# kssteven418/Q-ASR

Measured on AMD Instinct MI355X. Metric: RTFx (audio-sec/wall-sec) QuartzNet15x5 int8 bs32, higher is better.
Workload: dtype int8 (s8 x s8 -> i32 on MFMA; float64 fixed-point requant)

## Files before the change

profiles/phase_stamps.py:

```python
#!/usr/bin/env python3
import argparse
import ctypes as C
import json
import os
import sys

ROOT = os.path.dirname(os.path.dirname(os.path.abspath(__file__)))
sys.path.insert(0, os.path.join(ROOT, 'q-asr_amd'))
sys.path.insert(0, ROOT)
import numpy as np
import torch

ap = argparse.ArgumentParser()
ap.add_argument('--tile', type=int, default=32, choices=[32, 64, 128])
ap.add_argument('--gen', type=int, default=2)
ap.add_argument('--batch', type=int, default=32)
args = ap.parse_args()
from qasr import engine, pack, synth, topology

d = np.load(os.path.join(ROOT, 'tests/golden/net_quartznet_w8a8.npz'))
meta = json.loads(str(d['meta']))
cfg = topology.quartznet15x5()
sd = synth.make_state_dict(cfg, meta['seed'])
blob, pm = pack.pack_model(cfg, sd, d['act_min'], d['act_max'], 8, 8)
e = engine.Engine(blob, 0, tile=args.tile, sep_gen=getattr(args, "gen", 2))
B, T = args.batch, 512
x = torch.from_numpy(synth.make_features(B, 64, T, 1)).cuda()
lens = torch.full((B,), 500)
for _ in range(3):
    e.forward(x, lens)
torch.cuda.synchronize()
lib = engine.load_library()
buf = torch.zeros(32, dtype=torch.int64, device='cuda')
lib.qasr_debug_prof(C.c_void_p(buf.data_ptr()))
labels = e.op_labels()
seen = {}
for oi, lab in enumerate(labels):
    if lab.startswith('k_sep'):
        seen[lab] = oi
for lab, oi in seen.items():
    for _ in range(3):
        e.run_op(oi)
    torch.cuda.synchronize()
    st = buf.cpu().numpy()
    n = int(st[31])
    deltas = [int(st[i + 1] - st[i]) for i in range(n - 1)]
    print(f'{lab:34s} op {oi:3d} stamps {n:2d} total {int(st[n - 1] - st[0]):6d}  deltas {deltas}')
lib.qasr_debug_prof(C.c_void_p(0))
e.close()
```

q-asr_amd/csrc/qasr_sep2_impl.h:

```cpp
#pragma once
#include <algorithm>
#include <cstdio>
#include <cstdlib>
#include <type_traits>

#include "qasr_device.h"

namespace qasr {

typedef int v2i __attribute__((ext_vector_type(2)));
typedef unsigned char __attribute__((address_space(3))) lds_u8;
typedef unsigned __attribute__((address_space(3))) lds_u32;
typedef v2i __attribute__((address_space(3))) lds_v2i;
typedef v4i __attribute__((address_space(3))) lds_v4i;

#define SEP2_NT 512
#ifndef SEP2_WPE
#define SEP2_WPE 2
#endif
#define SEP2_CH 128

template <int K, int TT>
struct Sep2Geo {
  static constexpr int PAD = K / 2;
  static constexpr int HALO = (PAD + 15) / 16 * 16;
  static constexpr int D = HALO - PAD;
  static constexpr int NU = TT / 16;
  static constexpr int S = 4 * NU;
  static constexpr int MS = -(D & 3);
  static constexpr int NS = (K + 3 - MS + 3) / 4;
  static constexpr int A0 = D + MS;
  static constexpr int RG = S < 16 ? S : 16;
  static constexpr int OFF = (A0 & (RG - 1)) / 4;
  static constexpr int NE = OFF + NU + NS - 1;
  static constexpr int NRD = (4 * NE + RG - 1) / RG;
  static constexpr int WLEN = TT + 2 * HALO;
#ifndef SEP2_CF128
#define SEP2_CF128 1
#endif
  static constexpr int WP = (TT > 64 && !SEP2_CF128) ? WLEN : ((WLEN + 4 * S - 1) / (4 * S) | 1) * (4 * S);
  static constexpr int NPG = WLEN / 16;
  static constexpr int NPT = (16 * NPG + 63) / 64;
  static constexpr int KP4 = (K + 3) / 4;
  static constexpr int KS = 4 * KP4 + 32;
  static constexpr int TAPB = 16 * KS;
  static constexpr int NTT = (KS + 63) / 64;
  static constexpr int WREG = 16 * WP + TAPB + 64;
  static_assert(3 * S + (A0 & ~(RG - 1)) + NRD * RG <= WLEN && WLEN <= WP, "lane stream leaves the window row");
  static_assert(8 + MS - 3 >= 0 && 8 + MS + 4 * (NS + 1) <= KS, "tap stream leaves the tap row");
  static_assert(WREG % 16 == 0, "wave regions are not 16-byte granular");
};

__device__ __forceinline__ int rq_clamp(int z, double M, int lo, int hi) { return med3i(rq_rint(z, M), lo, hi); }
__device__ __forceinline__ unsigned pack4b(int a, int b, int c, int d) {
  const unsigned lo = __builtin_amdgcn_perm((unsigned)b, (unsigned)a, 0x0c0c0400u);
  const unsigned hi = __builtin_amdgcn_perm((unsigned)d, (unsigned)c, 0x04000c0cu);
  return lo | hi;
}

__device__ __forceinline__ int sep2_a_lane_off(int lane) {
  return (16 * (lane >> 5) + ((lane & 15) >> 1)) * 32 + 16 * ((lane >> 4) & 1) + 8 * (lane & 1);
}
__device__ __forceinline__ v4i sep2_a_frag(const lds_u8* img_lane, int ks) {
  const v2i lo = __builtin_amdgcn_ds_read_tr8_b64_v2i32((lds_v2i*)(img_lane + ks * 1024));
  const v2i hi = __builtin_amdgcn_ds_read_tr8_b64_v2i32((lds_v2i*)(img_lane + ks * 1024 + 256));
  return (v4i){lo[0], lo[1], hi[0], hi[1]};
}
__device__ __forceinline__ void sep2_load_wg(v4i* wb, const v4i* __restrict__ wp) {
#pragma unroll
  for (int i = 0; i < 4; ++i) wb[i] = wp[64 * i];
}
template <int MT, int N, int N0>
__device__ __forceinline__ void sep2_gemm(v16i (&acc)[MT], v4i (&wf)[16], const lds_u8* img_lane, int mt_stride,
                                          const v4i* __restrict__ r0, const v4i* __restrict__ r1) {
  constexpr int AB = MT > 2 ? 1 : 2;
  constexpr int NQ = 4 * N / AB;
  v4i a[2][MT][AB];
#pragma unroll
  for (int mt = 0; mt < MT; ++mt)
#pragma unroll
    for (int i = 0; i < AB; ++i) a[0][mt][i] = sep2_a_frag(img_lane + mt * mt_stride, i);
#pragma unroll
  for (int q = 0; q < NQ; ++q) {
    if (q + 1 < NQ) {
#pragma unroll
      for (int mt = 0; mt < MT; ++mt)
#pragma unroll
        for (int i = 0; i < AB; ++i) a[(q + 1) & 1][mt][i] = sep2_a_frag(img_lane + mt * mt_stride, AB * (q + 1) + i);
    }
#pragma unroll
    for (int i = 0; i < AB; ++i)
#pragma unroll
      for (int mt = 0; mt < MT; ++mt)
        acc[mt] = __builtin_amdgcn_mfma_i32_32x32x32_i8(a[q & 1][mt][i], wf[AB * q + i], acc[mt], 0, 0, 0);
    if ((AB * (q + 1)) % 4 == 0) {
      const int g = (AB * (q + 1)) / 4 - 1;
      if (g < N0) {
        if (r0) sep2_load_wg(&wf[4 * g], r0 + 256 * g);
      } else {
        if (r1) sep2_load_wg(&wf[4 * g], r1 + 256 * g);
      }
    }
  }
}

template <int D, int NE, int RG>
__device__ __forceinline__ void sep2_rd_stream(unsigned* xs, const lds_u8* wr) {
  if constexpr (D < NE) {
    constexpr int n = (RG == 16 && D % 4 == 0 && NE - D >= 4) ? 4 : (D % 2 == 0 && NE - D >= 2) ? 2 : 1;
    if constexpr (n == 4) {
      const v4i v = *(const lds_v4i*)(wr + 4 * D);
      xs[D] = v[0]; xs[D + 1] = v[1]; xs[D + 2] = v[2]; xs[D + 3] = v[3];
    } else if constexpr (n == 2) {
      const v2i v = *(const lds_v2i*)(wr + 4 * D);
      xs[D] = v[0]; xs[D + 1] = v[1];
    } else {
      xs[D] = *(const lds_u32*)(wr + 4 * D);
    }
    sep2_rd_stream<D + n, NE, RG>(xs, wr);
  }
}

__device__ __forceinline__ v4i sep2_mask16(v4i pk, int n) {
#pragma unroll
  for (int i = 0; i < 4; ++i) {
    const int m = min(max(n - 4 * i, 0), 4);
    pk[i] &= m >= 4 ? -1 : (int)((1u << (8 * m)) - 1u);
  }
  return pk;
}
template <int MT>
__device__ __forceinline__ bool sep2_any_wide(const v16i (&a)[MT]) {
  int mx = a[0][0], mn = a[0][0];
#pragma unroll
  for (int mt = 0; mt < MT; ++mt)
#pragma unroll
    for (int r = 0; r < 16; r += 2) {
      mx = max(max(mx, a[mt][r]), a[mt][r + 1]);
      mn = min(min(mn, a[mt][r]), a[mt][r + 1]);
    }
  return __any(mx >= (1 << 21) || mn < -(1 << 21));
}

template <int I, int N, class F>
__device__ __forceinline__ void sep2_for(F&& f) {
  if constexpr (I < N) {
    f(std::integral_constant<int, I>{});
    sep2_for<I + 1, N>(f);
  }
}
template <int MT, int N, int N0, int AB, class CB>
__device__ __forceinline__ void sep2_gemm_cb(v16i* __restrict__ acc, v4i (&wf)[16], const lds_u8* img_lane, int mt_stride,
                                             const v4i* __restrict__ r0, const v4i* __restrict__ r1, CB&& cb) {
  constexpr int NQ = 4 * N / AB;
  v4i a[2][MT][AB];
#pragma unroll
  for (int mt = 0; mt < MT; ++mt)
#pragma unroll
    for (int i = 0; i < AB; ++i) a[0][mt][i] = sep2_a_frag(img_lane + mt * mt_stride, i);
  sep2_for<0, NQ>([&](auto qc) {
    constexpr int q = decltype(qc)::value;
    if constexpr (q + 1 < NQ) {
#pragma unroll
      for (int mt = 0; mt < MT; ++mt)
#pragma unroll
        for (int i = 0; i < AB; ++i) a[(q + 1) & 1][mt][i] = sep2_a_frag(img_lane + mt * mt_stride, AB * (q + 1) + i);
    }
    sep2_for<0, AB * MT>([&](auto sc) {
      constexpr int sl = decltype(sc)::value, i = sl / MT, mt = sl % MT;
      acc[mt] = __builtin_amdgcn_mfma_i32_32x32x32_i8(a[q & 1][mt][i], wf[AB * q + i], acc[mt], 0, 0, 0);
      __builtin_amdgcn_sched_barrier(0);
      cb(std::integral_constant<int, q * AB * MT + sl>{});
      __builtin_amdgcn_sched_barrier(0);
    });
    if constexpr ((AB * (q + 1)) % 4 == 0) {
      constexpr int g = (AB * (q + 1)) / 4 - 1;
      if constexpr (g < N0) {
        if (r0) sep2_load_wg(&wf[4 * g], r0 + 256 * g);
      } else {
        if (r1) sep2_load_wg(&wf[4 * g], r1 + 256 * g);
      }
    }
    __builtin_amdgcn_sched_barrier(0);
  });
}

template <int MT, int J0, int NJ, class CB>
__device__ __forceinline__ void sep2_gemm_ks(v16i* __restrict__ acc, v4i (&wf)[16], const lds_u8* img_lane, int mt_stride, CB&& cb) {
  v4i a[2][MT];
#pragma unroll
  for (int mt = 0; mt < MT; ++mt) a[0][mt] = sep2_a_frag(img_lane + mt * mt_stride, J0);
  sep2_for<0, NJ>([&](auto qc) {
    constexpr int q = decltype(qc)::value;
    if constexpr (q + 1 < NJ) {
#pragma unroll
      for (int mt = 0; mt < MT; ++mt) a[(q + 1) & 1][mt] = sep2_a_frag(img_lane + mt * mt_stride, J0 + q + 1);
    }
    sep2_for<0, MT>([&](auto mc) {
      constexpr int mt = decltype(mc)::value;
      acc[mt] = __builtin_amdgcn_mfma_i32_32x32x32_i8(a[q & 1][mt], wf[J0 + q], acc[mt], 0, 0, 0);
      __builtin_amdgcn_sched_barrier(0);
      cb(std::integral_constant<int, q * MT + mt>{});
      __builtin_amdgcn_sched_barrier(0);
    });
    __builtin_amdgcn_sched_barrier(0);
  });
}

#define SEP2_PAIR_HALF 32768
#define SEP2_PAIR_SPIN 400000
typedef unsigned v4u __attribute__((ext_vector_type(4)));
typedef v4u __attribute__((address_space(3))) lds_v4u;
typedef unsigned __attribute__((address_space(1))) glb_u32;
__device__ __forceinline__ void sep2_pair_signal(unsigned* flag, int tid) {
  asm volatile("s_waitcnt vmcnt(0)" ::: "memory");
  __syncthreads();
  if (tid == 0) (void)__hip_atomic_fetch_add((glb_u32*)flag, 1u, __ATOMIC_RELAXED, __HIP_MEMORY_SCOPE_AGENT);
}
__device__ __forceinline__ void sep2_pair_wait(unsigned* flag, unsigned* tmo, int wave, int lane) {
  if (wave == 0) {
    const unsigned long long t_end = __builtin_amdgcn_s_memrealtime() + SEP2_PAIR_SPIN;
    while (__hip_atomic_load((glb_u32*)flag, __ATOMIC_RELAXED, __HIP_MEMORY_SCOPE_AGENT) == 0u) {
      __builtin_amdgcn_s_sleep(2);
      if (__builtin_amdgcn_s_memrealtime() > t_end) {
        if (lane == 0) (void)__hip_atomic_fetch_add((glb_u32*)tmo, 1u, __ATOMIC_RELAXED, __HIP_MEMORY_SCOPE_AGENT);
        break;
      }
    }
  }
  __builtin_amdgcn_fence(__ATOMIC_ACQUIRE, "wavefront");
  __syncthreads();
}

struct Sep2PassP {
  int bias, pbias;
  double Mo[QASR_MAX_OUTS];
  double Mm, Mp;
  float sbm, sbp;
};

template <int K, int NG, int NGP, int NP, bool DBG, int TT, int DIL = 1, bool SKIP = false, bool PAIR = false>
__device__ __forceinline__ void sep2_body(const SepP& p, const int b, const int t0, const bool stamp_wg, const int wg_id,
                                          const int hm = 0, const int pair_id = 0) {
  using G = Sep2Geo<K, TT / DIL>;
  constexpr bool RES = NGP > 0;
  static_assert(!PAIR || (K > 0 && NG == 4 && NGP == 0 && NP == 2 && !DBG && TT == 128 && DIL == 1 && !SKIP),
                "paired form: the plain 512 -> 512 layers at 128 frames");
  constexpr int NPL = PAIR ? 1 : NP;
  const int cbase = PAIR ? 256 * hm : 0;
  static_assert(DIL == 1 || (DIL == 2 && !RES && TT >= 64), "dilation 2: plain layers, 64- / 128-frame tiles");
  constexpr int MT = TT / 32;
  constexpr int NU = G::NU, S = G::S, NS = G::NS;
  constexpr int CIN_PAD = 128 * NG, PCIN_PAD = 128 * NGP;
  constexpr int RCH = 16 / DIL, GCH = SEP2_CH / DIL;
  constexpr int NCHUNK = PAIR ? 2 : (CIN_PAD + GCH - 1) / GCH;
  constexpr int NPGR = DIL == 1 ? G::NPG : (TT + 2 * DIL * G::HALO) / 16;
  constexpr int NPT = (RCH * NPGR + 63) / 64, NTG = RCH * G::KS / 16, NTT = (NTG + 63) / 64;
  static_assert(DIL == 1 || (8 * NPGR == G::WLEN && (RCH * G::KS) % 16 == 0), "dilation 2: window / tap granules");
  extern __shared__ __attribute__((aligned(16))) unsigned char smem[];
  const EpiP& e = p.e;
  int tid_ = threadIdx.x;
  asm volatile("" : "+v"(tid_));
  const int tid = tid_, lane = tid & 63, h = lane >> 5;
  const int wave = __builtin_amdgcn_readfirstlane(tid >> 6);
  lds_u8* const Xd = (lds_u8*)smem;
  lds_u8* const Un = Xd + TT * CIN_PAD;
  lds_u8* const Wsw = Un + wave * G::WREG;
  lds_u8* const Tlw = Wsw + 16 * G::WP;

  const unsigned flags = e.flags;
  const int eT = e.T, eTp = e.Tp, ecout = e.cout, n_outs = e.n_outs;
  const int len_b = e.lens[b];
  const int lim = (flags & QASR_F_MASK_OUT) ? min(len_b, eT) : eT;
  const int dlim = min(len_b, eT);
  const bool f_relu = flags & QASR_F_RELU;
  const bool f_exact = flags & QASR_F_EXACT_Z;
  int dw_lo = p.dw_lo, dw_hi = p.dw_hi;
  asm volatile("" : "+v"(dw_lo), "+v"(dw_hi));
  const bool stamp = p.prof && (p.prof_mode & 255) == 0 && stamp_wg && tid == 0;
  const bool tline = p.prof && (p.prof_mode & 255) == 1 && tid == 0;
  const int tune = p.prof_mode >> 8;
  long long tl_start = 0, tl_clk = 0;
  if (tline) {
    tl_start = (long long)__builtin_amdgcn_s_memrealtime();
    tl_clk = (long long)__builtin_amdgcn_s_memtime();
  }
  int nst = 0;
#define STAMP2() do { if (stamp && nst < 31) p.prof[nst++] = (long long)__builtin_amdgcn_s_memtime(); } while (0)
  STAMP2();

  const unsigned flip = p.x_unsigned ? 0x80808080u : 0u;
  constexpr int NRT = RES ? (TT * PCIN_PAD / 16) / SEP2_NT : 0;
  v4i pc[NPT], pt[NTT], rr[NRT > 0 ? NRT : 1], wf[16];
  const int co_l = 32 * wave + (lane & 31);
  const v4i* const w0 = w_frag(p.w, CIN_PAD, cbase + co_l, 0);
  const v4i* const w0a = PAIR ? w0 + 64 * 8 * hm : w0;
  const v4i* const w0b = PAIR ? w0 + 64 * 8 * (1 - hm) - 64 * 8 : w0;
  int woff[NPT], toff[NTT];
  unsigned wkeep[NPT];
  lds_u8* wlds[NPT];
#pragma unroll
  for (int i = 0; i < NPT; ++i) {
    const int pi = lane + 64 * i;
    const int row = pi / NPGR, col = pi - row * NPGR;
    const int t = t0 - DIL * G::HALO + 16 * col;
    woff[i] = min(row, RCH - 1) * eTp + min(max(t, 0), eTp - 16);
    wkeep[i] = (t >= 0 && t < eTp) ? 0xffffffffu : 0u;
    wlds[i] = DIL == 1 ? Wsw + min(row, 15) * G::WP + 16 * col : Wsw + 2 * min(row, RCH - 1) * G::WP + 8 * col;
    asm volatile("" : "+v"(wkeep[i]));
  }
#pragma unroll
  for (int i = 0; i < NTT; ++i) toff[i] = 16 * min(lane + 64 * i, NTG - 1);
  auto ld_grp = [&](int g) {
    const int cw = cbase + GCH * g + RCH * wave;
    const int8_t* const xg = p.x + ((size_t)b * CIN_PAD + cw) * eTp;
    const unsigned char* const tg = (const unsigned char*)p.wdw2 + (size_t)cw * G::KS;
#pragma unroll
    for (int i = 0; i < NPT; ++i) pc[i] = *(const v4i*)(xg + woff[i]);
#pragma unroll
    for (int i = 0; i < NTT; ++i) pt[i] = *(const v4i*)(tg + toff[i]);
  };
  auto ld_res = [&](int i) {
    if constexpr (RES) {
      const int gi = tid + SEP2_NT * i;
      const int c = gi / (TT / 16), q = gi - c * (TT / 16);
      rr[i] = *(const v4i*)(p.panes[0].x + ((size_t)b * PCIN_PAD + c) * eTp + t0 + 16 * q);
    }
  };
  constexpr int SLC = NCHUNK >= 4 ? 3 : PAIR ? 2 : 1;
  auto pf = [&](auto chc, int lo, int hi) {
    constexpr int CH = decltype(chc)::value;
    constexpr int n_res = CH + 1 == NCHUNK ? NRT : 0;
    constexpr int s0 = CH < SLC ? 4 * NG * CH / SLC : 0, n_slab = CH < SLC ? 4 * NG * (CH + 1) / SLC - s0 : 0;
#pragma unroll
    for (int i = lo; i < hi; ++i) {
      if (i < n_res) ld_res(i);
      else if (i < n_res + n_slab) wf[s0 + i - n_res] = (s0 + i - n_res < 8 ? w0a : w0b)[64 * (s0 + i - n_res)];
    }
  };
  auto commit = [&]() {
#pragma unroll
    for (int i = 0; i < NPT; ++i) {
      if (64 * i + 63 < RCH * NPGR || lane + 64 * i < RCH * NPGR) {
        v4i v = pc[i];
        v[0] = (v[0] & wkeep[i]) ^ flip; v[1] = (v[1] & wkeep[i]) ^ flip; v[2] = (v[2] & wkeep[i]) ^ flip; v[3] = (v[3] & wkeep[i]) ^ flip;
        if constexpr (DIL == 1) {
          *(lds_v4i*)wlds[i] = v;
        } else {
          const v2i ev = {(int)__builtin_amdgcn_perm((unsigned)v[1], (unsigned)v[0], 0x06040200u),
                          (int)__builtin_amdgcn_perm((unsigned)v[3], (unsigned)v[2], 0x06040200u)};
          const v2i od = {(int)__builtin_amdgcn_perm((unsigned)v[1], (unsigned)v[0], 0x07050301u),
                          (int)__builtin_amdgcn_perm((unsigned)v[3], (unsigned)v[2], 0x07050301u)};
          *(lds_v2i*)wlds[i] = ev;
          *(lds_v2i*)(wlds[i] + G::WP) = od;
        }
      }
    }
#pragma unroll
    for (int i = 0; i < NTT; ++i) {
      const int gi = lane + 64 * i;
      if (64 * i + 63 < NTG || gi < NTG) *(lds_v4i*)(Tlw + 16 * gi) = pt[i];
    }
  };
  constexpr int NXT = K == 0 ? (TT * CIN_PAD / 16) / SEP2_NT : 1;
  v4i xg[NXT];
  if constexpr (K == 0) {
#pragma unroll
    for (int i = 0; i < NXT; ++i) {
      const int gi = tid + SEP2_NT * i;
      const int c = gi / (TT / 16), q = gi - c * (TT / 16);
      xg[i] = *(const v4i*)(p.x + ((size_t)b * CIN_PAD + c) * eTp + t0 + 16 * q);
    }
#pragma unroll
    for (int j = 0; j < 4 * NG; ++j) wf[j] = w0[64 * j];
  } else {
    ld_grp(0);
  }
  STAMP2();

  const int cb = lane >> 2, jl = lane & 3;
  int dbias[NCHUNK];
  double dM[NCHUNK];
  if constexpr (K > 0) {
#pragma unroll
    for (int gi = 0; gi < NCHUNK; ++gi) {
      const int c = cbase + GCH * gi + RCH * wave + cb / DIL;
      dbias[gi] = p.bias_dw[c];
      dM[gi] = p.m_dw[c];
    }
  }
  Sep2PassP pps[NPL];
  auto load_pps = [&]() {
#pragma unroll
  for (int ps = 0; ps < NPL; ++ps) {
    const int cor = cbase + 256 * ps + co_l;
    Sep2PassP& q = pps[ps];
    q.bias = p.bias[cor];
    if constexpr (RES) {
      q.pbias = p.panes[0].bias[cor];
      q.Mm = e.m_main[cor];
      q.Mp = p.panes[0].m[cor];
      q.sbp = f_exact ? p.panes[0].sb[cor] : 1.0f;
    } else {
#pragma unroll
      for (int j = 0; j < QASR_MAX_OUTS; ++j) q.Mo[j] = j < n_outs ? e.outs[j].mtab[cor] : 0.0;
    }
    q.sbm = f_exact ? e.sb[cor] : 1.0f;
  }
  };
  if constexpr (K == 0) load_pps();

  if constexpr (SKIP && !DBG) {
    asm volatile("" ::: "memory");
    if ((flags & QASR_F_MASK_OUT) && t0 >= lim && !p.prof) {
      store_masked_tile<SEP2_NT>(e, b, t0, TT, 0, ecout, tid);
      return;
    }
  }
  const bool full_in = t0 + TT <= dlim;
  constexpr int e0base = 8 + G::MS;
  const int e0 = e0base - jl, tq = e0 >> 2, tsh = e0 & 3;
  unsigned fmask[NU];
  {
    const int dl = dlim - t0 - S * jl;
#pragma unroll
    for (int u = 0; u < NU; ++u) {
      const int n = min(max(dl - 4 * u, 0), 4);
      fmask[u] = n >= 4 ? 0xffffffffu : ((1u << (8 * n)) - 1u);
    }
  }
  struct DwIn {
    unsigned raw[NS + 1];
    unsigned xs[G::NRD * (G::RG / 4)];
  };
  const lds_u32* tr_lane = (const lds_u32*)(Tlw + (cb / DIL) * G::KS + 4 * tq);
  const lds_u8* wr_lane = Wsw + cb * G::WP + S * jl + (G::A0 & ~(G::RG - 1));
  asm volatile("" : "+v"(tr_lane), "+v"(wr_lane));
  auto dw_read = [&](DwIn& in) {
    const lds_u32* tr = tr_lane;
#pragma unroll
    for (int i = 0; i <= NS; ++i) in.raw[i] = tr[i];
    const lds_u8* wr = wr_lane;
    sep2_rd_stream<G::OFF, G::NE, G::RG>(in.xs, wr);
  };
  auto dw_mfma = [&](const DwIn& in, v4i (&acc)[NU], int bias, auto&& pf3) {
    unsigned tw[NS];
#pragma unroll
    for (int st = 0; st < NS; ++st) tw[st] = __builtin_amdgcn_alignbyte(in.raw[st + 1], in.raw[st], tsh);
#pragma unroll
    for (int u = 0; u < NU; ++u) acc[u] = (v4i){bias, bias, bias, bias};
    pf3(0);
#pragma unroll
    for (int st = 0; st < NS; ++st) {
      if (st == NS / 2) pf3(1);
#pragma unroll
      for (int u = 0; u < NU; ++u)
        acc[u] = __builtin_amdgcn_mfma_i32_4x4x4i8((int)tw[st], (int)in.xs[G::OFF + u + st], acc[u], 0, 0, 0);
    }
    pf3(2);
  };
  auto dw_out = [&](v4i (&acc)[NU], int c0, double Mg) {
    if constexpr (DIL == 2) {
      const int c = c0 + RCH * wave + (cb >> 1), par = cb & 1;
#pragma unroll
      for (int u = 0; u < NU; ++u)
#pragma unroll
        for (int v = 0; v < 4; ++v) {
          const int f = 2 * (S * jl + 4 * u + v) + par;
          if (DBG && p.dw_acc_dbg && t0 + f < eT) p.dw_acc_dbg[((size_t)b * CIN_PAD + c) * eTp + t0 + f] = acc[u][v];
          *(lds_u8*)(Xd + (f >> 5) * (CIN_PAD * 32) + c * 32 + (f & 31)) = (unsigned char)rq_clamp(acc[u][v], Mg, dw_lo, dw_hi);
        }
      return;
    }
    const int c = c0 + 16 * wave + cb;
    if (DBG && p.dw_acc_dbg) {
#pragma unroll
      for (int u = 0; u < NU; ++u)
#pragma unroll
        for (int v = 0; v < 4; ++v) {
          const int f = S * jl + 4 * u + v;
          if (t0 + f < eT) p.dw_acc_dbg[((size_t)b * CIN_PAD + c) * eTp + t0 + f] = acc[u][v];
        }
    }
#pragma unroll
    for (int u = 0; u < NU; ++u) {
      const int f = S * jl + 4 * u;
      const unsigned w = pack4b(rq_clamp(acc[u][0], Mg, dw_lo, dw_hi), rq_clamp(acc[u][1], Mg, dw_lo, dw_hi),
                                rq_clamp(acc[u][2], Mg, dw_lo, dw_hi), rq_clamp(acc[u][3], Mg, dw_lo, dw_hi));
      *(lds_u32*)(Xd + (f >> 5) * (CIN_PAD * 32) + c * 32 + (f & 31)) = w & fmask[u];
    }
  };

  auto dw_mfma_ilv = [&](const DwIn& in, v4i (&acc)[NU], int bias, auto&& pf3, v4i (&prev)[NU], int cprev, double Mprev) {
    constexpr int NOPS = 17 * NU, OPM = (NOPS + NS * NU - 1) / (NS * NU);
    const int c = cprev + 16 * wave + cb;
#pragma unroll
    for (int u = 0; u < NU; ++u) acc[u] = (v4i){bias, bias, bias, bias};
    unsigned tws[2] = {__builtin_amdgcn_alignbyte(in.raw[1], in.raw[0], tsh), 0u}, P1 = 0, P2 = 0;
    double dreg = 0.0;
    int q[4] = {0, 0, 0, 0};
    __builtin_amdgcn_sched_barrier(0);
    sep2_for<0, NS * NU>([&](auto ic) {
      constexpr int i = decltype(ic)::value, st = i / NU, u = i % NU;
      if constexpr (u == 0) {
        if constexpr (st == 0) pf3(0);
        if constexpr (st == NS / 2) pf3(1);
      }
      if constexpr (u == NU / 2 && st + 1 < NS) tws[(st + 1) & 1] = __builtin_amdgcn_alignbyte(in.raw[st + 2], in.raw[st + 1], tsh);
      acc[u] = __builtin_amdgcn_mfma_i32_4x4x4i8((int)tws[st & 1], (int)in.xs[G::OFF + u + st], acc[u], 0, 0, 0);
      sep2_for<OPM * i, OPM * (i + 1)>([&](auto jc) {
      constexpr int j = decltype(jc)::value;
      if constexpr (j < NOPS) {
        constexpr int dw = j / 17, r = j % 17;
        if constexpr (r < 12) {
          constexpr int val = r / 3, ph = r % 3;
          if constexpr (ph == 0) dreg = (double)prev[dw][val];
          if constexpr (ph == 1) dreg = __builtin_fma(dreg, Mprev, MAGIC_RNE);
          if constexpr (ph == 2) q[val] = med3i(__double2loint(dreg), dw_lo, dw_hi);
        } else if constexpr (r == 12) {
          P1 = __builtin_amdgcn_perm((unsigned)q[1], (unsigned)q[0], 0x0c0c0400u);
        } else if constexpr (r == 13) {
          P2 = __builtin_amdgcn_perm((unsigned)q[3], (unsigned)q[2], 0x04000c0cu);
        } else if constexpr (r == 14) {
          P1 |= P2;
        } else if constexpr (r == 15) {
          P1 &= fmask[dw];
        } else {
          constexpr int f0 = 4 * dw;
          const int f = S * jl + f0;
          *(lds_u32*)(Xd + (f >> 5) * (CIN_PAD * 32) + c * 32 + (f & 31)) = P1;
        }
      }
      });
      __builtin_amdgcn_sched_barrier(0);
    });
    pf3(2);
  };

  DwIn in;
  auto stage = [&](auto chc) {
    constexpr int CH = decltype(chc)::value;
    commit();
    if constexpr (CH + 1 < NCHUNK) ld_grp(CH + 1);
    __builtin_amdgcn_fence(__ATOMIC_RELEASE, "wavefront");
    __builtin_amdgcn_wave_barrier();
    __builtin_amdgcn_fence(__ATOMIC_ACQUIRE, "wavefront");
    dw_read(in);
    __builtin_amdgcn_sched_barrier(0);
  };
#ifndef SEP2_ILV
#define SEP2_ILV 1
#endif
#ifndef SEP2_TAIL1
#define SEP2_TAIL1 0
#endif
  constexpr bool ILV = SEP2_ILV && (!RES || TT <= 64) && DIL == 1;
  v4i accs[ILV ? 2 : 1][NU];
  auto chunk = [&](auto chc) {
    constexpr int CH = decltype(chc)::value;
    constexpr int c0 = GCH * CH;
    constexpr int NPF = (CH + 1 == NCHUNK ? NRT : 0) + (CH < SLC ? 4 * NG * (CH + 1) / SLC - 4 * NG * CH / SLC : 0);
    constexpr int Q = (NPF + 2) / 3;
    if constexpr (ILV) {
      if constexpr (CH == 0) dw_mfma(in, accs[0], dbias[0], [&](int k) { pf(chc, Q * k, Q * (k + 1)); });
      else {
        if (DBG && p.dw_acc_dbg) {
          dw_out(accs[(CH - 1) & 1], c0 - GCH, dM[CH - 1]);
          dw_mfma(in, accs[CH & 1], dbias[CH], [&](int k) { pf(chc, Q * k, Q * (k + 1)); });
        } else {
          dw_mfma_ilv(in, accs[CH & 1], dbias[CH], [&](int k) { pf(chc, Q * k, Q * (k + 1)); }, accs[(CH - 1) & 1],
                      c0 - GCH, dM[CH - 1]);
        }
      }
      __builtin_amdgcn_sched_barrier(0);
      STAMP2();
      if constexpr (CH + 1 < NCHUNK) stage(std::integral_constant<int, CH + 1>{});
      else dw_out(accs[CH & 1], c0, dM[CH]);
      STAMP2();
    } else {
      dw_mfma(in, accs[0], dbias[CH], [&](int k) { pf(chc, Q * k, Q * (k + 1)); });
      STAMP2();
      if constexpr (CH + 1 < NCHUNK) stage(std::integral_constant<int, CH + 1>{});
      dw_out(accs[0], c0, dM[CH]);
      __builtin_amdgcn_sched_barrier(0);
      STAMP2();
    }
  };
  if constexpr (K > 0) {
    if (stamp) {
      asm volatile("s_waitcnt vmcnt(0)" ::: "memory");
      STAMP2();
    }
    if (tune & 1) {
      if (wave < 4) __builtin_amdgcn_s_setprio(3);
    }
    stage(std::integral_constant<int, 0>{});
    load_pps();
    if (tune & 2) {
      if (wave >= 4)
        for (int i = 0; i < ((tune >> 4) & 127); ++i) __builtin_amdgcn_s_sleep(1);
    }
    STAMP2();
    sep2_for<0, NCHUNK>([&](auto chc) { chunk(chc); });
  } else {
    static_assert(K > 0 || !RES, "the bare 1x1 form has no residual variant");
    const unsigned xflip = p.pw_unsigned ? 0x80808080u : 0u;
#pragma unroll
    for (int i = 0; i < NXT; ++i) {
      const int gi = tid + SEP2_NT * i;
      const int c = gi / (TT / 16), q = gi - c * (TT / 16);
      v4i v = xg[i];
      v[0] ^= xflip; v[1] ^= xflip; v[2] ^= xflip; v[3] ^= xflip;
      *(lds_v4i*)(Xd + (q >> 1) * (CIN_PAD * 32) + c * 32 + 16 * (q & 1)) = v;
    }
  }
  static_assert(NCHUNK <= 4 * DIL, "more than 512 input channels");
  if ((tune & 5) == 1) __builtin_amdgcn_s_setprio(0);
  __syncthreads();
  if constexpr (PAIR) {
    const auto rs = __builtin_amdgcn_make_buffer_rsrc(p.pair_x + ((size_t)pair_id * 2 + hm) * SEP2_PAIR_HALF, 0, SEP2_PAIR_HALF, 0x00020000);
#pragma unroll
    for (int i = 0; i < MT; ++i) {
      const v4u v = *(const lds_v4u*)(Xd + i * (CIN_PAD * 32) + tid * 16);
      __builtin_amdgcn_raw_buffer_store_b128(v, rs, i * (SEP2_PAIR_HALF / MT) + tid * 16, 0, 16);
    }
  }
  if constexpr (DIL == 2) {
    if (t0 + TT > dlim) {
      for (int r = tid; r < MT * CIN_PAD; r += SEP2_NT) {
        const int mt = r / CIN_PAD, n = dlim - t0 - 32 * mt;
        if (n < 32) {
          lds_v4i* row = (lds_v4i*)(Xd + (size_t)r * 32);
          row[0] = sep2_mask16(row[0], n);
          row[1] = sep2_mask16(row[1], n - 16);
        }
      }
      __syncthreads();
    }
  }
  if constexpr (RES) {
    const unsigned rflip = p.panes[0].x_unsigned ? 0x80808080u : 0u;
#pragma unroll
    for (int i = 0; i < NRT; ++i) {
      const int gi = tid + SEP2_NT * i;
      const int c = gi / (TT / 16), q = gi - c * (TT / 16);
      v4i v = rr[i];
      v[0] ^= rflip; v[1] ^= rflip; v[2] ^= rflip; v[3] ^= rflip;
      *(lds_v4i*)(Un + (q >> 1) * (PCIN_PAD * 32) + c * 32 + 16 * (q & 1)) = v;
    }
    __syncthreads();
  }
  STAMP2();
  const lds_u8* const xd_lane = Xd + sep2_a_lane_off(lane);
  const lds_u8* const xr_lane = Un + sep2_a_lane_off(lane);
  int32_t* const pdbg = RES ? p.panes[0].acc_dbg : nullptr;
  const int qlo = f_relu ? max(e.qlo, 0) : e.qlo, qhi = e.qhi;
  constexpr bool PIPED = !RES && (NP * (MT >= 2 ? 2 : 1) > 1);
  static_assert(!PAIR || PIPED, "paired form: the pipelined epilogue");
  if constexpr (PIPED) {
    {
      constexpr int MH = MT >= 2 ? MT / 2 : 1, NH = MT / MH;
      constexpr bool SPLIT = SEP2_TAIL1 && MH == 2;
      constexpr int NUN0 = NP * NH, NUN = NUN0 + (SPLIT ? 1 : 0);
      const OutP& o0 = e.outs[0];
      const int olo = o0.lo, ohi = o0.hi;
      int8_t* const optr = (int8_t*)o0.ptr;
      v16i accs[2][MH];
      int q4[4];
      unsigned P[4];
      auto unit_finish = [&](v16i* a, int ps, int mt0, auto mhc) __attribute__((always_inline)) {
        constexpr int mh = decltype(mhc)::value;
        const int co = cbase + 256 * ps + co_l;
        if (DBG && e.acc_dbg) {
#pragma unroll
          for (int mt = 0; mt < mh; ++mt)
#pragma unroll
            for (int r = 0; r < 16; ++r) {
              const int t = t0 + 32 * (mt0 + mt) + mfma32_row(r, h);
              if (t < eT) e.acc_dbg[((size_t)b * ecout + co) * eTp + t] = a[mt][r];
            }
        }
        if (f_exact) {
          int mx = a[0][0], mn = a[0][0];
#pragma unroll
          for (int mt = 0; mt < mh; ++mt)
#pragma unroll
            for (int r = 0; r < 16; r += 2) {
              mx = max(max(mx, a[mt][r]), a[mt][r + 1]);
              mn = min(min(mn, a[mt][r]), a[mt][r + 1]);
            }
          if (__any(mx >= (1 << 21) || mn < -(1 << 21))) {
#pragma unroll
            for (int mt = 0; mt < mh; ++mt)
#pragma unroll
              for (int r = 0; r < 16; ++r) a[mt][r] = z_roundtrip(a[mt][r], pps[ps].sbm, f_relu);
          }
        }
      };
      auto unit_values = [&](v16i* a, int ps, int mt0, auto v0c, auto v1c) __attribute__((always_inline)) {
        constexpr int v0 = decltype(v0c)::value, v1 = decltype(v1c)::value;
        sep2_for<v0, v1>([&](auto vc) {
          constexpr int v = decltype(vc)::value, mt = v / 16, r = v % 16;
          q4[r & 3] = rq_clamp(a[mt][r], pps[ps].Mo[0], olo, ohi);
          if constexpr ((r & 3) == 3) P[r >> 2] = pack4b(q4[0], q4[1], q4[2], q4[3]);
          if constexpr (r == 15) {
            const auto s02 = __builtin_amdgcn_permlane32_swap(P[0], P[2], false, false);
            const auto s13 = __builtin_amdgcn_permlane32_swap(P[1], P[3], false, false);
            v4i pk = {(int)s02[0], (int)s02[1], (int)s13[0], (int)s13[1]};
            if (t0 + 32 * (mt0 + mt + 1) > lim) pk = sep2_mask16(pk, lim - (t0 + 32 * (mt0 + mt) + 16 * h));
            *(v4i*)(optr + ((size_t)b * ecout + cbase + 256 * ps + co_l) * eTp + t0 + 32 * (mt0 + mt) + 16 * h) = pk;
          }
        });
      };
      auto u_ps = [](int u) constexpr { return u < NUN0 ? u / NH : NP - 1; };
      auto u_mh = [](int u) constexpr { return (SPLIT && u >= NUN0 - 1) ? 1 : MH; };
      auto u_mt0 = [](int u) constexpr { return u < NUN0 ? (u % NH) * MH : (NH - 1) * MH + 1; };
      if constexpr (PAIR) {
        static_assert(MH == 2 && NH == 2 && !SPLIT, "paired form: two units of two tiles");
        using mh2 = std::integral_constant<int, 2>;
#pragma unroll
        for (int un = 0; un < 2; ++un)
#pragma unroll
          for (int mt = 0; mt < 2; ++mt)
#pragma unroll
            for (int r = 0; r < 16; ++r) accs[un][mt][r] = pps[0].bias;
        auto none = [](auto) {};
        sep2_pair_signal(p.pair_flags + 2 * pair_id + hm, tid);
        STAMP2();
        sep2_gemm_ks<2, 0, 8>(accs[0], wf, xd_lane, CIN_PAD * 32, none);
        sep2_pair_wait(p.pair_flags + 2 * pair_id + (1 - hm), p.pair_tmo, wave, lane);
        v4u pv[MT];
        {
          const auto rs = __builtin_amdgcn_make_buffer_rsrc(p.pair_x + ((size_t)pair_id * 2 + (1 - hm)) * SEP2_PAIR_HALF, 0, SEP2_PAIR_HALF, 0x00020000);
#pragma unroll
          for (int i = 0; i < MT; ++i) pv[i] = __builtin_amdgcn_raw_buffer_load_b128(rs, i * (SEP2_PAIR_HALF / MT) + tid * 16, 0, 16);
        }
        __builtin_amdgcn_sched_barrier(0);
        sep2_gemm_ks<2, 0, 8>(accs[1], wf, xd_lane + 2 * (CIN_PAD * 32), CIN_PAD * 32, none);
        STAMP2();
#pragma unroll
        for (int i = 0; i < MT; ++i) *(lds_v4u*)(Xd + i * (CIN_PAD * 32) + SEP2_PAIR_HALF / MT + tid * 16) = pv[i];
        __syncthreads();
        STAMP2();
        sep2_gemm_ks<2, 8, 8>(accs[0], wf, xd_lane, CIN_PAD * 32, none);
        unit_finish(accs[0], 0, 0, mh2{});
        sep2_gemm_ks<2, 8, 8>(accs[1], wf, xd_lane + 2 * (CIN_PAD * 32), CIN_PAD * 32, [&](auto qc) {
          constexpr int q = decltype(qc)::value;
          unit_values(accs[0], 0, 0, std::integral_constant<int, 2 * q>{}, std::integral_constant<int, 2 * q + 2>{});
        });
        STAMP2();
        unit_finish(accs[1], 0, 2, mh2{});
        unit_values(accs[1], 0, 2, std::integral_constant<int, 0>{}, std::integral_constant<int, 32>{});
        STAMP2();
      } else {
      sep2_for<0, NUN>([&](auto uc) {
        constexpr int u = decltype(uc)::value, ps = u_ps(u), mh = u_mh(u), mt0 = u_mt0(u);
        constexpr int AB = mh >= 2 ? 1 : 2, NSL = 4 * NG * mh;
        v16i* const cur = accs[u & 1];
#pragma unroll
        for (int mt = 0; mt < mh; ++mt)
#pragma unroll
          for (int r = 0; r < 16; ++r) cur[mt][r] = pps[ps].bias;
        const v4i* const wnext = (u < NUN0 && u % NH == NH - 1 && ps + 1 < NP) ? w_frag(p.w, CIN_PAD, 256 * (ps + 1) + co_l, 0) : nullptr;
        if constexpr (u > 0) unit_finish(accs[(u - 1) & 1], u_ps(u - 1), u_mt0(u - 1), std::integral_constant<int, u_mh(u - 1)>{});
        sep2_gemm_cb<mh, NG, 0, AB>(cur, wf, xd_lane + mt0 * (CIN_PAD * 32), CIN_PAD * 32, nullptr, wnext, [&](auto qc) {
          if constexpr (u > 0) {
            constexpr int NV = 16 * u_mh(u - 1), VPS = (NV + NSL - 1) / NSL;
            constexpr int q = decltype(qc)::value, v0 = q * VPS < NV ? q * VPS : NV, v1 = (q + 1) * VPS < NV ? (q + 1) * VPS : NV;
            unit_values(accs[(u - 1) & 1], u_ps(u - 1), u_mt0(u - 1), std::integral_constant<int, v0>{}, std::integral_constant<int, v1>{});
          }
        });
        STAMP2();
      });
      unit_finish(accs[(NUN - 1) & 1], NP - 1, u_mt0(NUN - 1), std::integral_constant<int, u_mh(NUN - 1)>{});
      unit_values(accs[(NUN - 1) & 1], NP - 1, u_mt0(NUN - 1), std::integral_constant<int, 0>{}, std::integral_constant<int, 16 * u_mh(NUN - 1)>{});
      STAMP2();
      }
    }
  }
  if constexpr (!PIPED) {
#pragma unroll
  for (int ps = 0; ps < NP; ++ps) {
    const int cbase = 256 * ps;
    const int co = cbase + co_l, cor = co;
    constexpr bool co_ok = true;
    const bool more = ps + 1 < NP;
    const v4i* const wnext = more ? w_frag(p.w, CIN_PAD, co + 256, 0) : nullptr;
    const v4i* const wpane = RES ? w_frag(p.panes[0].w, PCIN_PAD, cor, 0) : nullptr;
    const Sep2PassP& pp = pps[ps];
    v16i acc[MT];
#pragma unroll
    for (int mt = 0; mt < MT; ++mt)
#pragma unroll
      for (int r = 0; r < 16; ++r) acc[mt][r] = pp.bias;
    if constexpr (RES) sep2_gemm<MT, NG, (NGP < NG ? NGP : NG)>(acc, wf, xd_lane, CIN_PAD * 32, wpane, wnext);
    else sep2_gemm<MT, NG, 0>(acc, wf, xd_lane, CIN_PAD * 32, nullptr, wnext);
    STAMP2();
    auto finish = [&](v16i (&a)[MT], int32_t* dbg, float sb) {
      if (DBG && dbg && co_ok) {
#pragma unroll
        for (int mt = 0; mt < MT; ++mt)
#pragma unroll
          for (int r = 0; r < 16; ++r) {
            const int t = t0 + 32 * mt + mfma32_row(r, h);
            if (t < eT) dbg[((size_t)b * ecout + co) * eTp + t] = a[mt][r];
          }
      }
      if (f_exact) {
        if (sep2_any_wide<MT>(a)) {
#pragma unroll
          for (int mt = 0; mt < MT; ++mt)
#pragma unroll
            for (int r = 0; r < 16; ++r) a[mt][r] = z_roundtrip(a[mt][r], sb, !RES && f_relu);
        }
      }
    };
    auto store16 = [&](void* optr, int mt, const int (&q)[16]) {
      unsigned P[4];
#pragma unroll
      for (int g = 0; g < 4; ++g) P[g] = pack4b(q[4 * g], q[4 * g + 1], q[4 * g + 2], q[4 * g + 3]);
      const auto s02 = __builtin_amdgcn_permlane32_swap(P[0], P[2], false, false);
      const auto s13 = __builtin_amdgcn_permlane32_swap(P[1], P[3], false, false);
      v4i pk = {(int)s02[0], (int)s02[1], (int)s13[0], (int)s13[1]};
      if (t0 + 32 * (mt + 1) > lim) pk = sep2_mask16(pk, lim - (t0 + 32 * mt + 16 * h));
      if (co_ok) *(v4i*)((int8_t*)optr + ((size_t)b * ecout + co) * eTp + t0 + 32 * mt + 16 * h) = pk;
    };

    if constexpr (RES) {
      finish(acc, e.acc_dbg, pp.sbm);
#pragma unroll
      for (int mt = 0; mt < MT; ++mt)
#pragma unroll
        for (int r = 0; r < 16; ++r) acc[mt][r] = rq_rint(acc[mt][r], pp.Mm);
      v16i accp[MT];
#pragma unroll
      for (int mt = 0; mt < MT; ++mt)
#pragma unroll
        for (int r = 0; r < 16; ++r) accp[mt][r] = pp.pbias;
      sep2_gemm<MT, NGP, (NGP < NG ? NGP : NG)>(accp, wf, xr_lane, PCIN_PAD * 32, wnext, nullptr);
      STAMP2();
      finish(accp, pdbg, pp.sbp);
#pragma unroll
      for (int mt = 0; mt < MT; ++mt) {
        int z[16];
#pragma unroll
        for (int r = 0; r < 16; ++r) z[r] = med3i(acc[mt][r] + rq_rint(accp[mt][r], pp.Mp), qlo, qhi);
#pragma unroll 1
        for (int j = 0; j < n_outs; ++j) {
          const OutP& o = e.outs[j];
          if (o.mode == 2) {
            store16(o.ptr, mt, z);
          } else {
            const double Mo = o.m;
            const int olo = o.lo, ohi = o.hi;
            int q[16];
#pragma unroll
            for (int r = 0; r < 16; ++r) q[r] = rq_clamp(z[r], Mo, olo, ohi);
            store16(o.ptr, mt, q);
          }
        }
      }
    } else {
      finish(acc, e.acc_dbg, pp.sbm);
#pragma unroll
      for (int j = 0; j < QASR_MAX_OUTS; ++j) {
        if (j < n_outs) {
          const OutP& o = e.outs[j];
          const int olo = o.lo, ohi = o.hi;
#pragma unroll
          for (int mt = 0; mt < MT; ++mt) {
            int q[16];
#pragma unroll
            for (int r = 0; r < 16; ++r) q[r] = rq_clamp(acc[mt][r], pp.Mo[j], olo, ohi);
            store16(o.ptr, mt, q);
          }
        }
      }
    }
    STAMP2();
  }
  }
  if (stamp) p.prof[31] = nst;
  if (tline && wg_id < p.prof_cap) {
    long long* r = p.prof + 4 * (size_t)wg_id;
    r[0] = tl_start;
    r[1] = (long long)__builtin_amdgcn_s_memrealtime();
    r[3] = (long long)__builtin_amdgcn_s_memtime() - tl_clk;
    r[2] = (long long)__builtin_amdgcn_s_getreg(63492) | ((long long)__builtin_amdgcn_s_getreg(6164) << 32);
  }
#undef STAMP2
}

template <int K, int NG, int NGP, int NP, bool DBG, int TT, int DIL = 1>
__global__ void __launch_bounds__(SEP2_NT, SEP2_WPE) k_sep2(SepP p) {
  sep2_body<K, NG, NGP, NP, DBG, TT, DIL>(p, blockIdx.x, blockIdx.y * TT, blockIdx.x == 0 && blockIdx.y == 1,
                                          blockIdx.y * gridDim.x + blockIdx.x);
}
template <int K, int NG, int NGP, int NP, int TT, int DIL = 1>
__global__ void __launch_bounds__(SEP2_NT, SEP2_WPE) k_sep2s(SepP p) {
  sep2_body<K, NG, NGP, NP, false, TT, DIL, true>(p, blockIdx.x, blockIdx.y * TT, blockIdx.x == 0 && blockIdx.y == 1,
                                                  blockIdx.y * gridDim.x + blockIdx.x);
}

template <int K>
__global__ void __launch_bounds__(SEP2_NT, SEP2_WPE) k_sep2p(SepP p) {
  const int id = blockIdx.x, P = 8 * (id >> 4) + (id & 7), hm = (id >> 3) & 1;
  const int B = p.e.B;
  if (P >= B * (p.e.Tp / 128)) return;
  const int t = P / B, b = P - t * B;
  sep2_body<K, 4, 0, 2, false, 128, 1, false, true>(p, b, t * 128, b == 0 && t == 1 && hm == 0, 2 * P + hm, hm, P);
}

template <int K, int TT, int DIL = 1>
static inline size_t sep2_smem_bytes(const SepP& p) {
  using G = Sep2Geo<K, TT / DIL>;
  const size_t xd = (size_t)TT * p.cin_pad;
  if (K == 0) return xd;
  size_t un = (size_t)(SEP2_NT / 64) * G::WREG;
  if (p.n_panes == 1) un = std::max(un, (size_t)TT * p.panes[0].cin_pad);
  return xd + un;
}

#define SEP2_INSTANCES(X) \
  X(33, 2, 0, 1) X(39, 2, 0, 1) X(51, 2, 0, 2) X(51, 4, 0, 2) X(63, 4, 0, 2) X(75, 4, 0, 2) \
  X(33, 2, 2, 1) X(39, 2, 2, 1) X(51, 4, 2, 2) X(51, 4, 4, 2) X(63, 4, 4, 2) X(75, 4, 4, 2) \
  X(0, 4, 0, 4)

static inline bool sep2_shape_ok(const SepP& p) {
  const EpiP& e = p.e;
  if (p.K < 0 || (p.dilation != 1 && p.dilation != 2) || p.dense_k > 1 || p.cin_pad & 127 || e.cout > 1024) return false;
  if (e.flags & (QASR_F_LOGITS | QASR_F_WIDE_RQ)) return false;
  if (e.n_outs < 1) return false;
  int ngp = 0;
  if (e.flags & QASR_F_RESADD) {
    if (p.n_panes != 1 || p.panes[0].cin_pad & 127) return false;
    ngp = p.panes[0].cin_pad >> 7;
    for (int j = 0; j < e.n_outs; ++j)
      if (e.outs[j].mode != 0 && e.outs[j].mode != 2) return false;
  } else {
    if (p.n_panes != 0 || e.n_outs != 1 || e.outs[0].mode != 1) return false;
  }
  if (p.cin != p.cin_pad || (e.cout & 255) || (ngp && p.panes[0].cin != p.panes[0].cin_pad)) return false;
  const int ng = p.cin_pad >> 7, np = (e.cout + 255) / 256;
  if (p.K > 0 && p.dilation == 2) return p.K == 87 && ng == 4 && ngp == 0 && np == 2;
#define SEP2_MATCH(K_, NG_, NGP_, NP_) if (p.K == K_ && ng == NG_ && ngp == NGP_ && np == NP_) return true;
  SEP2_INSTANCES(SEP2_MATCH)
#undef SEP2_MATCH
  return false;
}

template <int K, int NG, int NGP, int NP, bool DBG, int TT, int DIL = 1, bool SKIP = false>
static int launch_sep2_v(hipStream_t s, const SepP& p) {
  const size_t smem = sep2_smem_bytes<K, TT, DIL>(p);
  if (smem > 160 * 1024 || p.e.B < 1 || p.e.Tp % TT || !p.x || !p.w || (K > 0 && !p.wdw2)) return QASR_ERR_ARG;
  static int attr_dev = -1;
  int dev = 0;
  (void)hipGetDevice(&dev);
  if (attr_dev != dev) {
    if constexpr (SKIP) (void)hipFuncSetAttribute((const void*)k_sep2s<K, NG, NGP, NP, TT, DIL>, hipFuncAttributeMaxDynamicSharedMemorySize, 160 * 1024);
    else (void)hipFuncSetAttribute((const void*)k_sep2<K, NG, NGP, NP, DBG, TT, DIL>, hipFuncAttributeMaxDynamicSharedMemorySize, 160 * 1024);
    attr_dev = dev;
  }
  SepP q = p;
  q.prof = g_prof;
  static const int tune = getenv("QASR_SEP2_TUNE") ? atoi(getenv("QASR_SEP2_TUNE")) : 0;
  q.prof_mode = g_prof_mode | (tune << 8);
  q.prof_cap = g_prof_cap;
  if constexpr (SKIP) hipLaunchKernelGGL((k_sep2s<K, NG, NGP, NP, TT, DIL>), dim3(p.e.B, p.e.Tp / TT, 1), dim3(SEP2_NT), smem, s, q);
  else hipLaunchKernelGGL((k_sep2<K, NG, NGP, NP, DBG, TT, DIL>), dim3(p.e.B, p.e.Tp / TT, 1), dim3(SEP2_NT), smem, s, q);
  return QASR_OK;
}

static inline bool sep2_pair_shape(const SepP& p) {
  return (p.K == 51 || p.K == 63 || p.K == 75) && p.dilation == 1 && p.cin_pad == 512 && p.e.cout == 512 && p.n_panes == 0 &&
         !(p.e.flags & QASR_F_RESADD) && p.e.Tp % 128 == 0;
}
static inline size_t sep2_pair_flag_bytes(int B, int Tp) { return ((size_t)B * (Tp / 128) * 2 * sizeof(unsigned) + 255) / 256 * 256; }
static inline size_t sep2_pair_x_bytes(int B, int Tp) { return (size_t)B * (Tp / 128) * 2 * SEP2_PAIR_HALF; }

template <int K>
static int launch_sep2_pair_v(hipStream_t s, const SepP& p) {
  const size_t smem = sep2_smem_bytes<K, 128, 1>(p);
  if (smem > 160 * 1024 || p.e.B < 1 || p.e.Tp % 128 || !p.x || !p.w || !p.wdw2 || !p.pair_flags || !p.pair_tmo || !p.pair_x) return QASR_ERR_ARG;
  static int attr_dev = -1;
  int dev = 0;
  (void)hipGetDevice(&dev);
  if (attr_dev != dev) {
    (void)hipFuncSetAttribute((const void*)k_sep2p<K>, hipFuncAttributeMaxDynamicSharedMemorySize, 160 * 1024);
    attr_dev = dev;
  }
  SepP q = p;
  q.prof = g_prof;
  q.prof_mode = g_prof_mode;
  q.prof_cap = g_prof_cap;
  const int npairs = p.e.B * (p.e.Tp / 128);
  hipLaunchKernelGGL((k_sep2p<K>), dim3(16 * ((npairs + 7) / 8)), dim3(SEP2_NT), smem, s, q);
  return QASR_OK;
}
int launch_sep2_pair(hipStream_t s, const SepP& p);

template <int TT, bool DBG, bool SKIP = false>
int launch_sep2_inst(hipStream_t s, const SepP& p) {
  const int ng = p.cin_pad >> 7, ngp = (p.e.flags & QASR_F_RESADD) ? (p.panes[0].cin_pad >> 7) : 0, np = (p.e.cout + 255) / 256;
  if (p.K > 0 && p.dilation == 2) {
    if constexpr (TT >= 64) {
      if (p.K == 87 && ng == 4 && ngp == 0 && np == 2) return launch_sep2_v<87, 4, 0, 2, DBG, TT, 2, SKIP>(s, p);
    }
    return QASR_ERR_UNSUPPORTED;
  }
#define SEP2_LAUNCH(K_, NG_, NGP_, NP_)                                                  \
  if constexpr (TT <= 64 || K_ > 0) {          \
    if (p.K == K_ && ng == NG_ && ngp == NGP_ && np == NP_) return launch_sep2_v<K_, NG_, NGP_, NP_, DBG, TT, 1, SKIP>(s, p); \
  }
  SEP2_INSTANCES(SEP2_LAUNCH)
#undef SEP2_LAUNCH
  return QASR_ERR_UNSUPPORTED;
}

}
```

Baseline: 297,400.

## Reorder separable-conv kernel prologue to issue loads before lane-constant math

Adds an EARLY mode, on by default, that forces every kernel argument into scalar registers in one round up front. The first input group load is issued before the per-lane window constants and the length-derived limits are computed. The pass-parameter loads and the second group prefetch are deferred until after the first MFMA step, so the first chunk's global latency overlaps setup work rather than serialising behind it. It also adds optional prologue timestamps and JSON output to the profiling script, at the cost of more code paths and extra register pressure from hoisted scalars.

```diff
diff --git a/profiles/phase_stamps.py b/profiles/phase_stamps.py
--- a/profiles/phase_stamps.py
+++ b/profiles/phase_stamps.py
@@ -15,6 +15,9 @@
 ap.add_argument('--tile', type=int, default=32, choices=[32, 64, 128])
 ap.add_argument('--gen', type=int, default=2)
 ap.add_argument('--batch', type=int, default=32)
+ap.add_argument('--prologue', action='store_true')
+ap.add_argument('--json')
+ap.add_argument('--tag', default='run')
 args = ap.parse_args()
 from qasr import engine, pack, synth, topology
 
@@ -34,17 +37,36 @@
 buf = torch.zeros(32, dtype=torch.int64, device='cuda')
 lib.qasr_debug_prof(C.c_void_p(buf.data_ptr()))
 labels = e.op_labels()
+paired = e.op_paired()
 seen = {}
 for oi, lab in enumerate(labels):
     if lab.startswith('k_sep'):
-        seen[lab] = oi
+        seen[lab + (' paired' if paired[oi] else '')] = oi
+PRO = ('start', 'arguments', 'constants', 'group0_requested', 'dw_params_requested', 'group0_back', 'rows_to_lds', 'first_mfma')
+rec = {}
 for lab, oi in seen.items():
+    buf.zero_()
     for _ in range(3):
         e.run_op(oi)
     torch.cuda.synchronize()
     st = buf.cpu().numpy()
     n = int(st[31])
     deltas = [int(st[i + 1] - st[i]) for i in range(n - 1)]
-    print(f'{lab:34s} op {oi:3d} stamps {n:2d} total {int(st[n - 1] - st[0]):6d}  deltas {deltas}')
+    print(f'{lab:41s} op {oi:3d} stamps {n:2d} total {int(st[n - 1] - st[0]):6d}  deltas {deltas}')
+    rec[lab] = dict(op=oi, total=int(st[n - 1] - st[0]), deltas=deltas)
+    if args.prologue and st[29]:
+        t = dict(start=st[0], arguments=st[24], constants=st[25], group0_requested=st[1], dw_params_requested=st[26],
+                 group0_back=st[2], rows_to_lds=st[27], first_mfma=st[3])
+        if lab.startswith('k_sep2<0,'):
+            t = dict(start=st[0], arguments=st[24], constants=st[25], group0_requested=st[1], dw_params_requested=st[26])
+        pro = {k: int(t[k] - st[29]) for k in PRO if k in t and t[k]}
+        print(f'{"":41s} prologue, cycles from the first instruction: {pro}')
+        rec[lab]['prologue'] = pro
+if args.json:
+    doc = json.load(open(args.json)) if os.path.exists(args.json) else {}
+    doc.setdefault('phase_stamps', {})[args.tag] = dict(tile=args.tile, batch=args.batch, lib=os.environ.get('QASR_LIB', 'default'),
+                                                        GPU_MAX_HW_QUEUES=os.environ.get('GPU_MAX_HW_QUEUES'), kernels=rec)
+    with open(args.json, 'w') as fh:
+        json.dump(doc, fh, indent=1)
 lib.qasr_debug_prof(C.c_void_p(0))
 e.close()
diff --git a/q-asr_amd/csrc/qasr_sep2_impl.h b/q-asr_amd/csrc/qasr_sep2_impl.h
--- a/q-asr_amd/csrc/qasr_sep2_impl.h
+++ b/q-asr_amd/csrc/qasr_sep2_impl.h
@@ -19,6 +19,12 @@
 #define SEP2_WPE 2
 #endif
 #define SEP2_CH 128
+#ifndef SEP2_EARLY
+#define SEP2_EARLY 1
+#endif
+#ifndef SEP2_PSTAMP
+#define SEP2_PSTAMP 0
+#endif
 
 template <int K, int TT>
 struct Sep2Geo {
@@ -239,6 +245,18 @@
   float sbm, sbp;
 };
 
+template <bool RES>
+__device__ __forceinline__ void sep2_args_round(const SepP& p) {
+  const EpiP& e = p.e;
+  asm volatile("" :: "s"(e.lens), "s"(e.Tp), "s"(e.B), "s"(p.x), "s"(p.wdw2), "s"(p.bias_dw), "s"(p.m_dw), "s"(p.prof), "s"(p.prof_mode),
+               "s"(p.dw_lo), "s"(p.dw_hi), "s"(e.flags), "s"(e.n_outs), "s"(p.x_unsigned), "s"(p.bias), "s"(e.sb), "s"(p.w));
+  if constexpr (RES) asm volatile("" :: "s"(p.panes[0].bias), "s"(e.m_main), "s"(p.panes[0].m), "s"(p.panes[0].sb),
+                                  "s"(p.panes[0].x_unsigned), "s"(p.panes[0].w), "s"(p.panes[0].x));
+  else asm volatile("" :: "s"(p.pw_unsigned), "s"(e.outs[0].mtab), "s"(e.outs[1].mtab), "s"(e.outs[2].mtab), "s"(e.outs[0].ptr),
+                    "s"(e.outs[0].lo), "s"(e.outs[0].hi));
+  __builtin_amdgcn_sched_barrier(0);
+}
+
 template <int K, int NG, int NGP, int NP, bool DBG, int TT, int DIL = 1, bool SKIP = false, bool PAIR = false>
 __device__ __forceinline__ void sep2_body(const SepP& p, const int b, const int t0, const bool stamp_wg, const int wg_id,
                                           const int hm = 0, const int pair_id = 0) {
@@ -268,15 +286,25 @@
   lds_u8* const Wsw = Un + wave * G::WREG;
   lds_u8* const Tlw = Wsw + 16 * G::WP;
 
+  long long t_entry = 0;
+  if constexpr (SEP2_PSTAMP != 0) {
+    t_entry = (long long)__builtin_amdgcn_s_memtime();
+    asm volatile("" : "+s"(t_entry) :: "memory");
+  }
   const unsigned flags = e.flags;
   const int eT = e.T, eTp = e.Tp, ecout = e.cout, n_outs = e.n_outs;
-  const int len_b = e.lens[b];
-  const int lim = (flags & QASR_F_MASK_OUT) ? min(len_b, eT) : eT;
-  const int dlim = min(len_b, eT);
+  constexpr bool EARLY = SEP2_EARLY && !SKIP;
+  if constexpr (EARLY && !DBG && !PAIR) sep2_args_round<(NGP > 0)>(p);
+  int len_b = e.lens[b], lim = 0, dlim = 0;
+  auto len_use = [&]() {
+    lim = (flags & QASR_F_MASK_OUT) ? min(len_b, eT) : eT;
+    dlim = min(len_b, eT);
+  };
+  if constexpr (!EARLY) len_use();
   const bool f_relu = flags & QASR_F_RELU;
   const bool f_exact = flags & QASR_F_EXACT_Z;
   int dw_lo = p.dw_lo, dw_hi = p.dw_hi;
-  asm volatile("" : "+v"(dw_lo), "+v"(dw_hi));
+  if constexpr (!EARLY) asm volatile("" : "+v"(dw_lo), "+v"(dw_hi));
   const bool stamp = p.prof && (p.prof_mode & 255) == 0 && stamp_wg && tid == 0;
   const bool tline = p.prof && (p.prof_mode & 255) == 1 && tid == 0;
   const int tune = p.prof_mode >> 8;
@@ -286,8 +314,15 @@
     tl_clk = (long long)__builtin_amdgcn_s_memtime();
   }
   int nst = 0;
-#define STAMP2() do { if (stamp && nst < 31) p.prof[nst++] = (long long)__builtin_amdgcn_s_memtime(); } while (0)
+#define STAMP2() do { if (stamp && nst < (SEP2_PSTAMP ? 24 : 31)) p.prof[nst++] = (long long)__builtin_amdgcn_s_memtime(); } while (0)
+#define PSTAMP2(I, WAIT) do { if constexpr (SEP2_PSTAMP != 0) { if (stamp) {                                   \
+      if (WAIT) asm volatile("s_waitcnt vmcnt(0) lgkmcnt(0)" ::: "memory");                                   \
+      p.prof[24 + (I)] = (long long)__builtin_amdgcn_s_memtime(); } } } while (0)
   STAMP2();
+  PSTAMP2(0, !EARLY);
+  if constexpr (SEP2_PSTAMP != 0) {
+    if (stamp) p.prof[24 + 5] = t_entry;
+  }
 
   const unsigned flip = p.x_unsigned ? 0x80808080u : 0u;
   constexpr int NRT = RES ? (TT * PCIN_PAD / 16) / SEP2_NT : 0;
@@ -299,18 +334,24 @@
   int woff[NPT], toff[NTT];
   unsigned wkeep[NPT];
   lds_u8* wlds[NPT];
-#pragma unroll
-  for (int i = 0; i < NPT; ++i) {
-    const int pi = lane + 64 * i;
-    const int row = pi / NPGR, col = pi - row * NPGR;
-    const int t = t0 - DIL * G::HALO + 16 * col;
-    woff[i] = min(row, RCH - 1) * eTp + min(max(t, 0), eTp - 16);
-    wkeep[i] = (t >= 0 && t < eTp) ? 0xffffffffu : 0u;
-    wlds[i] = DIL == 1 ? Wsw + min(row, 15) * G::WP + 16 * col : Wsw + 2 * min(row, RCH - 1) * G::WP + 8 * col;
-    asm volatile("" : "+v"(wkeep[i]));
-  }
-#pragma unroll
-  for (int i = 0; i < NTT; ++i) toff[i] = 16 * min(lane + 64 * i, NTG - 1);
+#define SEP2_LANE_CONSTS(OFFS, REST)                                                                                     \
+  _Pragma("unroll") for (int i = 0; i < NPT; ++i) {                                                                      \
+    const int pi = lane + 64 * i;                                                                                        \
+    const int row = pi / NPGR, col = pi - row * NPGR;                                                                    \
+    const int t = t0 - DIL * G::HALO + 16 * col;                  \
+                                                           \
+    if constexpr (OFFS) woff[i] = min(row, RCH - 1) * eTp + min(max(t, 0), eTp - 16);                                    \
+    if constexpr (REST) {                                                                                                \
+      wkeep[i] = (t >= 0 && t < eTp) ? 0xffffffffu : 0u;                        \
+                     \
+      wlds[i] = DIL == 1 ? Wsw + min(row, 15) * G::WP + 16 * col : Wsw + 2 * min(row, RCH - 1) * G::WP + 8 * col;        \
+      asm volatile("" : "+v"(wkeep[i]));                      \
+    }                                                                                                                    \
+  }                                                                                                                      \
+  if constexpr (OFFS) {                                                                                                  \
+    _Pragma("unroll") for (int i = 0; i < NTT; ++i) toff[i] = 16 * min(lane + 64 * i, NTG - 1);                          \
+  }
+  SEP2_LANE_CONSTS(true, !EARLY)
   auto ld_grp = [&](int g) {
     const int cw = cbase + GCH * g + RCH * wave;
     const int8_t* const xg = p.x + ((size_t)b * CIN_PAD + cw) * eTp;
@@ -374,9 +415,15 @@
 #pragma unroll
     for (int j = 0; j < 4 * NG; ++j) wf[j] = w0[64 * j];
   } else {
+    if constexpr (!EARLY) PSTAMP2(1, false);
     ld_grp(0);
   }
   STAMP2();
+  if constexpr (EARLY) {
+    SEP2_LANE_CONSTS(false, true)
+    asm volatile("" : "+v"(dw_lo), "+v"(dw_hi));
+    PSTAMP2(1, false);
+  }
 
   const int cb = lane >> 2, jl = lane & 3;
   int dbias[NCHUNK];
@@ -389,6 +436,12 @@
       dM[gi] = p.m_dw[c];
     }
   }
+  if constexpr (EARLY) {
+    asm volatile("" : "+v"(len_b));
+    len_b = __builtin_amdgcn_readfirstlane(len_b);
+    len_use();
+  }
+  PSTAMP2(2, false);
   Sep2PassP pps[NPL];
   auto load_pps = [&]() {
 #pragma unroll
@@ -541,12 +594,15 @@
   auto stage = [&](auto chc) {
     constexpr int CH = decltype(chc)::value;
     commit();
-    if constexpr (CH + 1 < NCHUNK) ld_grp(CH + 1);
+    if constexpr (CH == 0) PSTAMP2(3, false);
+    constexpr bool RD1ST = EARLY && CH == 0;
+    if constexpr (CH + 1 < NCHUNK && !RD1ST) ld_grp(CH + 1);
     __builtin_amdgcn_fence(__ATOMIC_RELEASE, "wavefront");
     __builtin_amdgcn_wave_barrier();
     __builtin_amdgcn_fence(__ATOMIC_ACQUIRE, "wavefront");
     dw_read(in);
     __builtin_amdgcn_sched_barrier(0);
+    if constexpr (CH + 1 < NCHUNK && RD1ST) ld_grp(CH + 1);
   };
 #ifndef SEP2_ILV
 #define SEP2_ILV 1
@@ -556,13 +612,16 @@
 #endif
   constexpr bool ILV = SEP2_ILV && (!RES || TT <= 64) && DIL == 1;
   v4i accs[ILV ? 2 : 1][NU];
+  auto pps_late = [&]() {
+    if constexpr (EARLY && !DBG) load_pps();
+  };
   auto chunk = [&](auto chc) {
     constexpr int CH = decltype(chc)::value;
     constexpr int c0 = GCH * CH;
     constexpr int NPF = (CH + 1 == NCHUNK ? NRT : 0) + (CH < SLC ? 4 * NG * (CH + 1) / SLC - 4 * NG * CH / SLC : 0);
     constexpr int Q = (NPF + 2) / 3;
     if constexpr (ILV) {
-      if constexpr (CH == 0) dw_mfma(in, accs[0], dbias[0], [&](int k) { pf(chc, Q * k, Q * (k + 1)); });
+      if constexpr (CH == 0) dw_mfma(in, accs[0], dbias[0], [&](int k) { pf(chc, Q * k, Q * (k + 1)); if (k == 1) pps_late(); });
       else {
         if (DBG && p.dw_acc_dbg) {
           dw_out(accs[(CH - 1) & 1], c0 - GCH, dM[CH - 1]);
@@ -578,7 +637,7 @@
       else dw_out(accs[CH & 1], c0, dM[CH]);
       STAMP2();
     } else {
-      dw_mfma(in, accs[0], dbias[CH], [&](int k) { pf(chc, Q * k, Q * (k + 1)); });
+      dw_mfma(in, accs[0], dbias[CH], [&](int k) { pf(chc, Q * k, Q * (k + 1)); if (CH == 0 && k == 1) pps_late(); });
       STAMP2();
       if constexpr (CH + 1 < NCHUNK) stage(std::integral_constant<int, CH + 1>{});
       dw_out(accs[0], c0, dM[CH]);
@@ -595,7 +654,7 @@
       if (wave < 4) __builtin_amdgcn_s_setprio(3);
     }
     stage(std::integral_constant<int, 0>{});
-    load_pps();
+    if constexpr (!EARLY || DBG) load_pps();
     if (tune & 2) {
       if (wave >= 4)
         for (int i = 0; i < ((tune >> 4) & 127); ++i) __builtin_amdgcn_s_sleep(1);
@@ -889,6 +948,8 @@
     r[2] = (long long)__builtin_amdgcn_s_getreg(63492) | ((long long)__builtin_amdgcn_s_getreg(6164) << 32);
   }
 #undef STAMP2
+#undef PSTAMP2
+#undef SEP2_LANE_CONSTS
 }
 
 template <int K, int NG, int NGP, int NP, bool DBG, int TT, int DIL = 1>
@@ -904,6 +965,7 @@
 
 template <int K>
 __global__ void __launch_bounds__(SEP2_NT, SEP2_WPE) k_sep2p(SepP p) {
+  if constexpr (SEP2_EARLY) sep2_args_round<false>(p);
   const int id = blockIdx.x, P = 8 * (id >> 4) + (id & 7), hm = (id >> 3) & 1;
   const int B = p.e.B;
   if (P >= B * (p.e.Tp / 128)) return;
```

Result: faster. 301,400 (median of 6 runs) (+1.4%).
